# nauful/NLZM

Measured on AMD Instinct MI355X. Metric: compress MB/s, higher is better.
Workload: dtype u8; 1 GPU; enwik9 stand-in: 1000000000 B stream, -window:28; step = 41 launches of 8 chunks (40136704 B) of the stream; timed: bytes [200683520, 401367040) of 1000000000 (a prefix: the steps asked for end before the stream does); window_bits=28, batch_chunks=8, whole_stream=False

## Files before the change

### nlzm_amd/csrc/nlzm_core.h

```cpp
#pragma once

#include <stdint.h>

#ifndef NLZM_HD
#define NLZM_HD __host__ __device__ __forceinline__
#endif
#ifndef NLZM_HDN
#define NLZM_HDN __host__ __device__
#endif
#define NLZM_RARE(x) __builtin_expect(!!(x), 0)

namespace nlzm {

constexpr uint32_t kMatchMin = 2;
constexpr uint32_t kMatchMax = 264;
constexpr uint32_t kNice = 64;
constexpr uint32_t kParseMax = 4096;
constexpr uint32_t kNone = 0xFFFFFFFFu;

constexpr uint32_t kCtxCmd = 0;
constexpr uint32_t kCtxLitHi = 1;
constexpr uint32_t kCtxLitLo = 2;
constexpr uint32_t kCtxLenDirect = 18;
constexpr uint32_t kCtxLenExtHi = 19;
// ... 99 lines not shown
    uint32_t *cap_words; unsigned long long cap_cap, cap_lo, cap_hi; unsigned long long *cap_used;
    uint32_t workers;
    uint32_t batch_a0;
    uint32_t *bt_ready;
    uint32_t *bt_pairs;
    uint32_t bt_pstride;
    uint32_t *bt_ext;
    uint32_t *bt_ext_cur;
    uint32_t bt_ext_cap;
    uint32_t *bt_flag;
    const uint8_t *unc;
    const uint32_t *bin_off;
    const uint32_t *bin_pos;
    uint32_t nheads;
    uint32_t wthreads;
    const uint32_t *hot_of_bin;
    const uint32_t *hot_list;
    unsigned long long *hot_undo;
    uint32_t *bt_undo;
    uint32_t *abort_word;
    const uint32_t *progress;
    WorkerCounters *wcnt;
    uint32_t table_shape;
    uint32_t launch_par;
    uint32_t test_fail;
    void *hook_user;
};

NLZM_HD uint32_t match_min(uint32_t d)
{
// ... 131 lines not shown

struct BtView {
    const uint8_t *in;
    uint32_t *heads, *tree, *ready, *pairs;
    uint32_t batch_a0, bt_shift, wmask, tmask;
    uint32_t pstride = kBtMaxPairs;
    uint32_t *ext = nullptr, *ext_cur = nullptr;
    uint32_t ext_cap = 0;
    uint32_t *fail_word = nullptr;
};
NLZM_HD BtView bt_view(const Geom &g, const Globals &G)
{
    return BtView{ G.in, G.bt_heads, G.bt_tree, G.bt_ready, G.bt_pairs, G.batch_a0, g.bt_shift, g.wmask, g.bt_tmask,
                   G.bt_pstride, G.bt_ext, G.bt_ext_cur, G.bt_ext_cap, G.abort_word };
}
template <class IO>
NLZM_HD void ResultSink<IO>::operator()(uint32_t d, uint32_t l)
{
    if (!pairs || l <= best) return;
    best = l; best_d = d;
    const bool s0 = count == 0, s1 = count == 1, s2 = count == 2, s3 = count == 3;
    d0 = s0 ? d : d0; l0 = s0 ? l : l0; d1 = s1 ? d : d1; l1 = s1 ? l : l1;
    d2 = s2 ? d : d2; l2 = s2 ? l : l2; d3 = s3 ? d : d3; l3 = s3 ? l : l3;
    if (count >= 4) {
        uint32_t *q = bt_pair_ptr<IO>(pairs, view->pstride, view->ext, view->ext_cur, view->ext_cap, ext_idx, count);
        if (q) { IO::st_agent(q, d); IO::st_agent(q + 1, l); }
    }
    count++;
}

// ... 32 lines not shown
```

### nlzm_amd/csrc/nlzm_hip.cpp

```cpp
#include <hip/hip_runtime.h>
#include <dirent.h>
#include <unistd.h>

#include <stdarg.h>
#include <stdint.h>
#include <stdio.h>
#include <stdlib.h>
#include <string.h>

#include <array>
#include <mutex>
#include <thread>
#include <chrono>
#include <algorithm>
#include <vector>

#include "../../include/nlzm_hip.h"
#include "nlzm_core.h"
#include "nlzm_v2.h"

namespace nlzm {
void launch_rk_hash(const uint8_t *in, unsigned long long n, unsigned long long pos0, unsigned long long pos1,
                    uint32_t *out, hipStream_t st);
void launch_pipeline2(const Geom &g, const Globals &G, const v2::GlobalsV2 &V, uint32_t c0, uint32_t c1, uint32_t worker_blocks, hipStream_t st);
// ... 50 lines not shown
void blocks_close(DevState &D, bool drop_pool = false);
bool idle_block_pool_dropped();

inline uint32_t clampu(uint32_t v, uint32_t lo, uint32_t hi) { return v < lo ? lo : (v > hi ? hi : v); }

struct Pool {
    uint8_t *base = nullptr;
    size_t size = 0, used = 0;
    bool measuring = false;
};

struct Options {
    int64_t batch = 32;
    int64_t worker_blocks = 240;
    int64_t worker_threads = 128;
    int64_t hot_waves = 2;
    int64_t hot_min = 0;
    int64_t tbits_max = 34;
    int64_t block_threads = 320;
    int64_t block_hot_waves = 3;
    int64_t block_batch = 8;
    int64_t tbits_per = 4;
    int64_t keep_pool = 1;
    int64_t helper = 1;
    int64_t block_helper = 0;
    int64_t multi_same = 0;
    int64_t table_shape = 0;
    int64_t test_fail_launch = -1;
    int64_t test_fail_stream = 0;
    int64_t block_ext_blocks = -1;
    int64_t report = 0;
};

struct StreamConfig {
    bool in_set = false;
    uint32_t batch = 0;
    uint32_t worker_blocks = 0, worker_threads = 0;
    uint32_t nheads = 0;
    uint32_t hot_max = 0;
    uint32_t hot_min = 0;
    uint32_t t_bits = 0, m_bits = 0;
    uint32_t t_bitmap = 0;
    uint32_t pstride = kBtMaxPairs, ext_cap = 0;
    bool helper = false;
    uint32_t table_shape = 0;
    int64_t test_fail_launch = -1;
    unsigned long long rkhash_len = 0;
    unsigned long long syms_stride = 0, bits_stride = 0, frame_stride = 0;
};

struct LaunchSet {
    uint32_t *rkhash = nullptr, *bt_ready = nullptr, *bt_flag = nullptr, *abort_word = nullptr, *bin_off = nullptr, *bin_pos = nullptr,
// ... 225 lines not shown
    memset(&C.stats, 0, sizeof C.stats);
    memset(&C.tm, 0, sizeof C.tm);
    C.stats.in_bytes = n;
    StreamConfig &K = C.cfg;
    StreamBuffers &B = C.buf;
    K = StreamConfig{};
    K.in_set = C.pool != nullptr;
    K.batch = (uint32_t)(O.batch < 1 ? 1 : O.batch);
    if (g.nchunks && K.batch > g.nchunks) K.batch = g.nchunks;
    {
        const int64_t room = (int64_t)C.cu_count - (int64_t)pipeline2_role_blocks();
        if (room < 1) return set_err(NLZM_HIP_E_ARG, "device has %d CUs: the pipeline needs at least %u", C.cu_count, pipeline2_role_blocks() + 1);
        K.worker_blocks = (uint32_t)(O.worker_blocks > room ? room : (O.worker_blocks < 1 ? 1 : O.worker_blocks));
    }
    K.worker_threads = (uint32_t)O.worker_threads;
    {
        K.nheads = 1u << (32 - g.bt_shift);
        const unsigned long long lanes = (unsigned long long)K.worker_blocks * K.worker_threads;
        if (lanes < K.nheads) K.nheads = (uint32_t)lanes;
    }
    {
        int64_t hw = O.hot_waves;
        const int64_t spare = (512 - O.worker_threads) / 64;
        if (hw > spare) hw = spare;
        K.hot_max = hw > 0 ? (uint32_t)hw * K.worker_blocks : 0u;
    }
    K.hot_min = (uint32_t)O.hot_min; K.table_shape = (uint32_t)O.table_shape; K.test_fail_launch = O.test_fail_launch; K.helper = O.helper != 0;
    K.t_bits = prefilter_tbits(g, O.tbits_per, O.tbits_max);
    K.t_bitmap = prefilter_is_bitmap(g) ? 1u : 0u;
    K.pstride = K.in_set ? 32u : kBtMaxPairs;
// ... 115 lines not shown
    G.batch_a0 = (uint32_t)a0;
    {
        const unsigned long long lo = a0 > 1024 ? a0 - 1024 : 0;
        unsigned long long hi = a1 + g.feed + 256;
        if (hi + 255 > g.n) hi = g.n >= 255 ? g.n - 255 : 0;
        HIPCHK(hipEventRecord(ev[7], C.st));
        if (hi > lo && hi - lo > K.rkhash_len) return set_err(NLZM_HIP_E_ARG, "launch of %u chunks is larger than the stream was opened for", nb);
        G.rkhash = L.rkhash - lo;
        if (g.n >= 256 && hi > lo) launch_rk_hash(C.d_in, g.n, lo, hi, L.rkhash - lo, C.st);
    }
    HIPCHK(hipEventRecord(ev[5], C.st));
    {
        const unsigned long long cnt = a1 - a0;
        G.bt_ready = L.bt_ready; G.bt_pairs = B.bt_pairs; G.bt_flag = L.bt_flag; G.unc = L.unc;
        G.bt_pstride = K.pstride; G.bt_ext = B.bt_ext; G.bt_ext_cap = K.ext_cap; G.bt_ext_cur = &B.v2_hx->ext_cur;
        G.bin_off = L.bin_off; G.bin_pos = L.bin_pos; G.nheads = K.nheads; G.wthreads = K.worker_threads;
        G.abort_word = L.abort_word; G.wcnt = B.wcnt; G.bt_undo = B.bt_undo;
        HIPCHK(hipMemsetAsync(L.bt_ready, 0, cnt * 4 * kBtRec, C.st));
        HIPCHK(hipMemsetAsync(L.bt_flag, 0, cnt * 4, C.st));
        HIPCHK(hipMemsetAsync(L.abort_word, 0, 4, C.st));
        HIPCHK(hipMemsetAsync(L.bin_off, 0, (size_t)nb * (K.nheads + 1) * 4, C.st));
        launch_prefilter(C.d_in, g.n, (uint32_t)a0, (uint32_t)a1, g.wmask, K.t_bits, K.t_bitmap, K.m_bits, B.pf_T, B.pf_M, B.pf_h, B.pf_h2,
                         B.pf_c1, L.unc, C.st);
        launch_bin(C.d_in, g, c0, nb, K.nheads, L.bin_off, B.bin_cur, L.bin_pos, L.unc, (uint32_t)a0, C.st);
        if (K.hot_max) {
            const unsigned long long lpos = (unsigned long long)K.batch * g.chunk_size;
            const double by_pace = K.in_set ? (double)lpos / 480.0 : (C.last_launch_ms > 0 ? 24.0 * C.last_launch_ms : (double)lpos / 240.0);
            const uint32_t hot_min = K.hot_min > 0 ? K.hot_min : (uint32_t)(by_pace < 512 ? 512 : (by_pace > 1e9 ? 1e9 : by_pace));
            launch_hot_select(L.bin_off, nb, K.nheads, K.hot_max, hot_min, L.hot_of_bin, L.hot_list, B.wcnt, C.st);
            G.hot_of_bin = L.hot_of_bin; G.hot_list = L.hot_list; G.hot_undo = B.hot_undo;
        }
// ... 168 lines not shown
    fprintf(stderr, "finder: RK256 entries cut short by the uint16 length parameter that became the growing top entry: %llu; that ended exactly where another entry ends: %llu (%llu of them the nearer one)\n",
            P.prof[115], P.prof[116], P.prof[117]);
    fprintf(stderr, "finder: starts of nice regions whose segment the stage knew itself, ahead of the parser's word: %llu; that it had to wait for: %llu\n", P.prof[118], P.prof[119]);
    fprintf(stderr, "finder: worker results not there at the first look: %llu of positions whose call is the finder's decision (unc), %llu of others\n", P.prof[28], P.prof[29]);
    fprintf(stderr, "finder: blocks that had to wait for a worker result: %llu (%.0f cycles each); late results of hot bins' waves %llu, late results at lane 0 (the position the block before was cut at) %llu\n",
            P.prof[112], (double)P.prof[25] / (double)(P.prof[112] ? P.prof[112] : 1), P.prof[110], P.prof[111]);
    fprintf(stderr, "parser: waited for its record loader %llu times, the table stage %.0f positions ahead on average then\n", P.prof[26], (double)P.prof[27] / (double)(P.prof[26] ? P.prof[26] : 1));
    if (P.prof[96] || P.prof[100])
        fprintf(stderr, "helper parser: %llu jobs posted, %llu taken over (%llu nodes = %.1f %% of the positions), the parser stage waited %.0f cycles per position for it; "
                        "helper: %llu jobs seen, %llu done, %llu blocks (%.2f passes each), waited %.0f cycles per position for records\n",
                P.prof[96], P.prof[97], P.prof[98], 100.0 * P.prof[98] / n, P.prof[99] / n, P.prof[100], P.prof[101], P.prof[102],
                (double)P.prof[103] / (double)(P.prof[102] ? P.prof[102] : 1), P.prof[104] / n);
    if (P.prof[88]) fprintf(stderr, "finder sections (cycles/position, profile build): predict %.0f, own loads %.0f, HT rows %.0f, candidates + jobs %.0f, record + RK256 %.0f, "
                            "BT4 results (wait included) %.0f, verify %.0f, commit %.0f\n", P.prof[88] / n, P.prof[89] / n, P.prof[90] / n, P.prof[91] / n, P.prof[92] / n,
                            P.prof[93] / n, P.prof[94] / n, P.prof[95] / n);
    if (P.prof[44]) fprintf(stderr, "table stage sections (cycles/position summed over the waves, profile build): gather %.0f, scan %.0f, waiting for the carry %.0f, carry merge (the part in block order) %.0f, records %.0f\n",
                            P.prof[44] / n, P.prof[45] / n, P.prof[47] / n, P.prof[46] / n, P.prof[55] / n);
    if (P.prof[32]) {
        const double np = (double)(P.prof[13] ? P.prof[13] : 1);
        fprintf(stderr, "parser, cycles per pass (profile build): relax waves %.0f %.0f %.0f, probe wave %.0f (of it: sets that changed %.0f, mask fills %.0f), update %.0f, "
                        "barrier waits per wave %.0f %.0f %.0f %.0f; block end %.0f cycles/position\n",
                P.prof[32] / np, P.prof[33] / np, P.prof[34] / np, P.prof[35] / np, P.prof[43] / np, P.prof[41] / np, P.prof[40] / np,
                P.prof[36] / np, P.prof[37] / np, P.prof[38] / np, P.prof[39] / np, P.prof[42] / n);
        fprintf(stderr, "parser, cycles per pass by wave 0..7 (profile build): work");
        for (int w = 0; w < 8; w++) fprintf(stderr, " %.0f", P.prof[64 + w] / np);
        fprintf(stderr, " | barrier wait");
        for (int w = 0; w < 8; w++) fprintf(stderr, " %.0f", P.prof[72 + w] / np);
        fprintf(stderr, " | update");
        for (int w = 0; w < 8; w++) fprintf(stderr, " %.0f", P.prof[80 + w] / np);
        fprintf(stderr, "\n");
// ... 273 lines not shown

void nlzm_hip_block_placement(uint32_t nstreams, uint32_t blocks_per_stream, uint32_t workgroup, uint32_t *stream, uint32_t *local)
{
    uint32_t s = 0, l = 0;
    multi_block_of(nstreams * blocks_per_stream, blocks_per_stream, workgroup, s, l);
    if (stream) *stream = s;
    if (local) *local = l;
}

enum OptKind { kOptRange,
               kOptLanes,
               kOptFlag,
               kOptAny };
static const struct { const char *key; int64_t Options::*member; OptKind kind; int64_t lo, hi; } kOptions[] = {
    { "worker_blocks", &Options::worker_blocks, kOptRange, 1, 255 },
    { "hot_waves", &Options::hot_waves, kOptRange, 0, 6 },
    { "hot_min", &Options::hot_min, kOptRange, 0, 1 << 30 },
    { "worker_threads", &Options::worker_threads, kOptLanes, 64, 512 },
    { "block_worker_threads", &Options::block_threads, kOptLanes, 64, 512 },
    { "block_hot_waves", &Options::block_hot_waves, kOptRange, 0, 6 },
    { "prefilter_bits_per_position", &Options::tbits_per, kOptRange, 0, 8 },
    { "stage_report", &Options::report, kOptFlag, 0, 0 },
    { "parser_helper", &Options::helper, kOptFlag, 0, 0 },
    { "table_shape", &Options::table_shape, kOptRange, 0, 2 },
    { "multi_allow_same_device", &Options::multi_same, kOptFlag, 0, 0 },
    { "test_fail_launch", &Options::test_fail_launch, kOptAny, 0, 0 },
    { "test_fail_stream", &Options::test_fail_stream, kOptRange, 0, 63 },
    { "block_ext_blocks", &Options::block_ext_blocks, kOptAny, 0, 0 },
    { "block_parser_helper", &Options::block_helper, kOptFlag, 0, 0 },
    { "keep_block_pool", &Options::keep_pool, kOptFlag, 0, 0 },
// ... 779 lines not shown
```

### nlzm_amd/csrc/nlzm_kernels.hip

```cpp
#include <hip/hip_runtime.h>
#include <type_traits>
#include <cstddef>
#include <stdint.h>

#include "nlzm_core.h"
#include "nlzm_v2.h"

namespace nlzm {

#ifndef NLZM_LPW
#define NLZM_LPW 64
#endif
#ifndef NLZM_AHEAD
#define NLZM_AHEAD 3
#endif
constexpr uint32_t kAhead = NLZM_AHEAD;
constexpr uint32_t kEntryWords = 16;
union V2Lds {
    v2::FLds f; v2::TLds t; v2::PLds p;
    uint32_t wq[512 * kAhead * kEntryWords];
};
__shared__ V2Lds g_v2_lds;
}
namespace xw {
// ... 243 lines not shown
    }
    static __device__ __forceinline__ uint32_t ld_agent(const uint32_t *p)
    {
        return __hip_atomic_load(p, __ATOMIC_RELAXED, __HIP_MEMORY_SCOPE_AGENT);
    }
    static __device__ __forceinline__ uint32_t atomic_inc(uint32_t *p) { return __hip_atomic_fetch_add(p, 1u, __ATOMIC_RELAXED, __HIP_MEMORY_SCOPE_AGENT); }
    static __device__ __forceinline__ void drain() { asm volatile("s_waitcnt vmcnt(0)" ::: "memory"); }
    static __device__ __forceinline__ void st_quad(uint32_t *p, uint32_t a, uint32_t b, uint32_t c, uint32_t d)
    {
        typedef uint32_t u4 __attribute__((ext_vector_type(4)));
        const u4 v = { a, b, c, d };
        asm volatile("global_store_dwordx4 %0, %1, off sc1\n\ts_nop 1" :: "v"((__attribute__((address_space(1))) uint32_t *)p), "v"(v) : "memory");
    }
};

struct LaneSink {
    uint32_t *slot;
    uint32_t *pairs;
    uint32_t count = 0, best = 1, best_d = 0;
    uint32_t ext_idx = 0;
    __device__ __forceinline__ void put(const BtView &B, uint32_t d, uint32_t l)
    {
        best = l; best_d = d;
        if (count < 4) { slot[(2 * count) * 512] = d; slot[(2 * count + 1) * 512] = l; }
        else {
            uint32_t *q = bt_pair_ptr<LaneIO>(pairs, B.pstride, B.ext, B.ext_cur, B.ext_cap, ext_idx, count);
            if (q) { LaneIO::st_agent(q, d); LaneIO::st_agent(q + 1, l); }
        }
        count++;
    }
    __device__ __forceinline__ void publish(uint32_t *rec, uint32_t tests) const
    {
        if (count > 4) LaneIO::drain();
        const uint32_t d0 = count > 0 ? slot[0] : 0u, l0 = count > 0 ? slot[512] : 0u, d1 = count > 1 ? slot[2 * 512] : 0u, l1 = count > 1 ? slot[3 * 512] : 0u;
        const uint32_t d2 = count > 2 ? slot[4 * 512] : 0u, l2 = count > 2 ? slot[5 * 512] : 0u, d3 = count > 3 ? slot[6 * 512] : 0u, l3 = count > 3 ? slot[7 * 512] : 0u;
        LaneIO::st_quad(rec + 4, d0, l0, d1, kBtTag);
        LaneIO::st_quad(rec + 8, l1, d2, l2, kBtTag);
        LaneIO::st_quad(rec + 12, d3, l3, ext_idx, kBtTag);
        LaneIO::st_quad(rec, kBtReady | (tests << 9) | count, best_d, count ? best : 0u, 0u);
    }
};
constexpr uint32_t kUndoCap = 260;
__device__ __forceinline__ void bt_descent(const BtView &B, uint32_t a, uint32_t hidx, uint32_t max_len, bool keep, bool dry, uint32_t *undo,
                                           uint32_t &n_undo, LaneSink &sink, uint32_t &tests_out, uint32_t &cmp_out)
{
    const uint8_t *pa = B.in + a;
    uint32_t sp = B.heads[hidx];
    uint32_t nu = 0;
    if (keep) { *(unsigned long long *)undo = (0x80000000u | hidx) | ((unsigned long long)(dry ? a : sp) << 32); nu = 1; }
    if (!dry) B.heads[hidx] = a;
    uint32_t pend_l = (a & B.tmask) << 1, pend_r = pend_l + 1, len_l = 0, len_r = 0, tests = 0, cb = 0;
    uint32_t old_l = kNone, old_r = kNone;
    while (sp != kNone && a > sp && a - sp <= B.wmask && tests < 256) {
        tests++;
        const uint32_t pair = (sp & B.tmask) << 1;
        const uint8_t *ps = B.in + sp;
        const uint32_t init = umin(len_l, len_r);
        const unsigned long long pp = *(const unsigned long long *)(B.tree + pair);
        const unsigned long long x0 = load64u(ps + init), y0 = load64u(pa + init), d0 = x0 ^ y0;
        const unsigned long long x1 = load64u(ps + init + 8), y1 = load64u(pa + init + 8), d1 = x1 ^ y1;
        const uint32_t nb0 = d0 ? (uint32_t)__builtin_ctzll(d0) >> 3 : (d1 ? 8u + ((uint32_t)__builtin_ctzll(d1) >> 3) : 16u);
        uint32_t l = init + nb0;
        bool full = l >= max_len;
        const unsigned long long xs = nb0 < 8 ? x0 : x1, ys = nb0 < 8 ? y0 : y1;
        uint32_t sign = (uint32_t)(((xs >> (8 * (nb0 & 7u))) & 0xFF) < ((ys >> (8 * (nb0 & 7u))) & 0xFF));
        if (nb0 == 16 && !full) {
            for (;;) {
                const unsigned long long x = load64u(ps + l), y = load64u(pa + l), d = x ^ y;
                if (d) {
                    const uint32_t nb = (uint32_t)__builtin_ctzll(d) >> 3;
                    l += nb;
                    sign = (uint32_t)(((x >> (8 * nb)) & 0xFF) < ((y >> (8 * nb)) & 0xFF));
                    break;
                }
                l += 8;
                if (l >= max_len) break;
            }
            full = l >= max_len;
        }
        if (full) l = max_len;
        cb += (l - init) + (full ? 0u : 1u);
        const uint32_t pl = (uint32_t)pp, pr = (uint32_t)(pp >> 32), d = a - sp;
        if (l >= match_min(d) && l > sink.best) sink.put(B, d, l);
        if (full) {
            if (!dry) { B.tree[pend_l] = pl; B.tree[pend_r] = pr; }
            if (keep) {
                *(unsigned long long *)(undo + 2 * nu) = pend_l | ((unsigned long long)(dry ? pl : old_l) << 32);
                *(unsigned long long *)(undo + 2 * nu + 2) = pend_r | ((unsigned long long)(dry ? pr : old_r) << 32);
                nu += 2;
            }
            tests_out = tests; cmp_out = cb; n_undo = nu;
            return;
        }
        const bool right = sign != 0;
        const uint32_t slot = right ? pend_l : pend_r;
        if (!dry) B.tree[slot] = sp;
        if (keep) { *(unsigned long long *)(undo + 2 * nu) = slot | ((unsigned long long)(dry ? sp : (right ? old_l : old_r)) << 32); nu++; }
        pend_l = right ? pair + 1 : pend_l; pend_r = right ? pend_r : pair;
        old_l = right ? pr : old_l; old_r = right ? old_r : pl;
        len_r = right ? l : len_r; len_l = right ? len_l : l;
        sp = right ? pr : pl;
    }
    if (!dry) { B.tree[pend_r] = kNone; B.tree[pend_l] = kNone; }
    if (keep) {
        *(unsigned long long *)(undo + 2 * nu) = pend_r | ((unsigned long long)(dry ? kNone : old_r) << 32);
        *(unsigned long long *)(undo + 2 * nu + 2) = pend_l | ((unsigned long long)(dry ? kNone : old_l) << 32);
        nu += 2;
    }
    tests_out = tests; cmp_out = cb; n_undo = nu;
}

#ifndef NLZM_RISKY_AHEAD
#define NLZM_RISKY_AHEAD 0
#endif
constexpr uint32_t kPending = 0xFFFFFFFEu;
__device__ __forceinline__ uint32_t wave_max_u32(uint32_t v) { return (uint32_t)__builtin_amdgcn_readlane((int)xw::scan_max(v), 63); }
__device__ __forceinline__ void worker_role_hot(const Geom &g, const Globals &G, uint32_t c0, uint32_t c1, uint32_t bin, uint32_t hot_index)
{
    unsigned long long p0 = (unsigned long long)G.in, p1 = (unsigned long long)G.bt_heads, p2 = (unsigned long long)G.bt_tree,
                       p3 = (unsigned long long)G.bt_ready, p4 = (unsigned long long)G.bt_pairs, p5 = (unsigned long long)G.bt_flag,
                       p6 = (unsigned long long)G.hot_undo;
    uint32_t q0 = G.batch_a0, q2 = g.wmask, q3 = g.bt_tmask;
    asm volatile("" : "+s"(p0), "+s"(p1), "+s"(p2), "+s"(p3), "+s"(p4), "+s"(p5), "+s"(p6));
    asm volatile("" : "+s"(q0), "+s"(q2), "+s"(q3));
#define NLZM_AS_GLOBAL(T, x) ((T *)(__attribute__((address_space(1))) T *)(x))
// ... 355 lines not shown
    constexpr uint32_t kLpw = NLZM_LPW;
    const uint32_t lane_waves = (G.wthreads + kLpw - 1) / kLpw;
    if ((threadIdx.x >> 6) >= lane_waves) {
        if (!G.hot_list) return;
        const uint32_t k = ((threadIdx.x >> 6) - lane_waves) * wblocks + wblock;
        if (k >= G.hot_list[0]) return;
        worker_role_hot(g, G, c0, c1, G.hot_list[1 + k], k);
        return;
    }
    const uint32_t lane_in_block = (threadIdx.x >> 6) * kLpw + (threadIdx.x & 63u);
    const bool takes_bin = (threadIdx.x & 63u) < kLpw && lane_in_block < G.wthreads;
    const uint32_t gl = wblock * G.wthreads + (takes_bin ? lane_in_block : 0u);
    unsigned long long p0 = (unsigned long long)G.in, p1 = (unsigned long long)G.bt_heads, p2 = (unsigned long long)G.bt_tree,
                       p3 = (unsigned long long)G.bt_ready, p4 = (unsigned long long)G.bt_pairs;
    uint32_t q0 = G.batch_a0, q1 = g.bt_shift, q2 = g.wmask, q3 = g.bt_tmask;
    asm volatile("" : "+s"(p0), "+s"(p1), "+s"(p2), "+s"(p3), "+s"(p4));
    asm volatile("" : "+s"(q0), "+s"(q1), "+s"(q2), "+s"(q3));
#define NLZM_AS_GLOBAL(T, x) ((T *)(__attribute__((address_space(1))) T *)(x))
    BtView B{ NLZM_AS_GLOBAL(const uint8_t, p0), NLZM_AS_GLOBAL(uint32_t, p1), NLZM_AS_GLOBAL(uint32_t, p2), NLZM_AS_GLOBAL(uint32_t, p3),
              NLZM_AS_GLOBAL(uint32_t, p4), q0, q1, q2, q3 };
    B.pstride = G.bt_pstride; B.ext = G.bt_ext; B.ext_cur = G.bt_ext_cur; B.ext_cap = G.bt_ext_cap; B.fail_word = G.abort_word;
    uint32_t *const undo_base = NLZM_AS_GLOBAL(uint32_t, (unsigned long long)G.bt_undo) + (unsigned long long)gl * (kAhead * kUndoCap * 2);
#undef NLZM_AS_GLOBAL
    bool active = takes_bin && gl < G.nheads && !(G.hot_of_bin && G.hot_of_bin[gl < G.nheads ? gl : 0]);
    uint32_t c = c0;
    bool loaded = false;
    uint32_t i0 = 0, e0 = 0;
    uint32_t la_end = 0;
    unsigned long long n_calls = 0, n_tests = 0, n_cmp = 0, n_open = 0, n_wait = 0, n_cyc = 0, n_cyc_tests = 0, n_back = 0, n_redo = 0;
    uint32_t first = 0, nq = 0, head_a = 0;
    uint32_t *const my = (uint32_t *)&g_v2_lds + threadIdx.x;
    enum : uint32_t { kWa = 8, kWtests = 9, kWcmp = 10, kWcount = 11, kWbest = 12, kWbestd = 13, kWundo = 14, kWinfo = 15 };
    unsigned long long t_wait0 = 0;
    uint32_t idle = 0, prog_seen = 0;
    bool fail = false;

    while (__any(active)) {
        bool waiting = false;
        uint32_t job = 0, ja = 0, jh = 0, jlen = 0, jinfo = 0;
        if (active) {
            if (nq) {
                const uint32_t f = LaneIO::ld_agent(G.bt_flag + (head_a - G.batch_a0));
                const bool hdry = (my[(first * kEntryWords + kWinfo) * 512] >> 28) & 1u;
                if ((f == kFlagCall && !hdry) || (f == kFlagSkip && hdry)) {
                    for (uint32_t k = 0; k < kAhead; k++) {
                        uint32_t *e = my + (first * kEntryWords) * 512;
                        if (!((e[kWinfo * 512] >> 28) & 1u)) { n_calls++; n_tests += e[kWtests * 512]; n_cmp += e[kWcmp * 512]; }
                        first = first + 1 == kAhead ? 0u : first + 1; nq--;
                        if (!nq) break;
                        e = my + (first * kEntryWords) * 512;
                        const uint32_t ea = e[kWa * 512], einfo = e[kWinfo * 512];
                        if (!((einfo >> 28) & 1u)) {
                            LaneSink sk{ e, B.pairs + (unsigned long long)(ea - B.batch_a0) * (2 * B.pstride), e[kWcount * 512] & 0x1FFu, e[kWbest * 512], e[kWbestd * 512], e[kWcount * 512] >> 9 };
                            sk.publish(B.ready + (unsigned long long)(ea - B.batch_a0) * kBtRec, e[kWtests * 512]);
                        }
// ... 58 lines not shown
                }
            }
            if (!job && nq) {
                waiting = true;
                n_wait++;
                if ((++idle & 1023u) == 0) {
                    if (LaneIO::ld_agent(G.abort_word)) active = false;
                    const unsigned long long now = wall_clock64();
                    const uint32_t prog = G.progress ? LaneIO::ld_agent(G.progress) : 0u;
                    if (!t_wait0 || prog != prog_seen) { t_wait0 = now; prog_seen = prog; }
                    else if (now - t_wait0 > 3000000000ull) { fail = true; }
                }
            }
            if (fail) { LaneIO::st_agent(G.abort_word, 2u); active = false; job = 0; }
        }
        if (job) {
            const unsigned long long t0 = __builtin_readcyclecounter();
            const unsigned long long bi = ja - B.batch_a0;
            const uint32_t slot = first + nq >= kAhead ? first + nq - kAhead : first + nq;
            uint32_t *e = my + (slot * kEntryWords) * 512;
            LaneSink sink{ e, B.pairs + bi * (2 * B.pstride) };
            uint32_t tests = 0, cmpb = 0, nu = 0;
            const bool park = job == 2 && ((jinfo >> 28) & 1u);
            if (!park) bt_descent(B, ja, jh, jlen, job == 2, false, undo_base + slot * (kUndoCap * 2), nu, sink, tests, cmpb);
            if (job == 1) {
                sink.publish(B.ready + bi * kBtRec, tests);
                n_calls++; n_tests += tests; n_cmp += cmpb;
                n_cyc += __builtin_readcyclecounter() - t0; n_cyc_tests += tests;
            } else {
                if (!nq) { if (!park) sink.publish(B.ready + bi * kBtRec, tests); head_a = ja; t_wait0 = 0; idle = 0; }
                e[kWa * 512] = ja; e[kWtests * 512] = tests; e[kWcmp * 512] = cmpb; e[kWcount * 512] = sink.count | (sink.ext_idx << 9);
                e[kWbest * 512] = sink.best; e[kWbestd * 512] = sink.best_d; e[kWundo * 512] = nu; e[kWinfo * 512] = jinfo;
                nq++; if (!park) n_open++;
            }
        }
        if (!__any(active && !waiting)) __builtin_amdgcn_s_sleep(8);
    }
    if (nq) {
        atomicAdd(&G.wcnt->stuck_lanes, 1ull);
        atomicMax(&G.wcnt->stuck_pos_inv, (unsigned long long)(uint32_t)~head_a);
    }
    for (int m = 32; m >= 1; m >>= 1) {
        n_calls += __shfl_xor(n_calls, m, 64); n_tests += __shfl_xor(n_tests, m, 64); n_cmp += __shfl_xor(n_cmp, m, 64);
        n_open += __shfl_xor(n_open, m, 64); n_wait += __shfl_xor(n_wait, m, 64);
        n_cyc += __shfl_xor(n_cyc, m, 64); n_cyc_tests += __shfl_xor(n_cyc_tests, m, 64);
        n_back += __shfl_xor(n_back, m, 64); n_redo += __shfl_xor(n_redo, m, 64);
    }
    if ((threadIdx.x & 63) == 0) {
        atomicAdd(&G.wcnt->bt_calls, n_calls); atomicAdd(&G.wcnt->bt_tests, n_tests); atomicAdd(&G.wcnt->cmp_bytes, n_cmp);
// ... 243 lines not shown
```

### nlzm_amd/csrc/nlzm_v2.h

```cpp
#pragma once

#include "nlzm_core.h"
#include "xw.h"

namespace nlzm {
namespace v2 {

constexpr uint32_t kFtRing = 1u << 14;
constexpr uint32_t kFtStride = 16;
constexpr uint32_t kTpRing = 1u << 13;
constexpr uint32_t kMaxEdges = 32;
constexpr uint32_t kTpStride = 2 + 2 + 2 * kMaxEdges;
constexpr uint32_t kTpUniq = 2, kTpEdges = 4;
constexpr uint32_t kFrontMax = 264;
constexpr uint32_t kTfStride = 2 * kFrontMax;

constexpr uint32_t kFtBt = 8u, kFtTop = 16u;
struct Hx {
    alignas(128) uint32_t f_pos;
    alignas(128) uint32_t t_pos;
    alignas(128) uint32_t t_out;
    alignas(128) uint32_t p_pos;
    alignas(128) unsigned long long p_seg;
    alignas(128) uint32_t h_job;
// ... 122 lines not shown
    uint32_t reach_d = kNone;
    uint32_t s_active, s_d, s_end, s_seen;
    uint32_t rk_from, rk_to, rk_len, rk_end;
    uint32_t rk_cut = 0;
    uint32_t prev_nice, seg_s;
    uint32_t gap_last = 0;
    uint32_t n_seg_own = 0, n_seg_wait = 0;
    uint32_t t_pos_seen;
    uint32_t err;
    uint32_t dbg_a = 0;
    unsigned long long n_pos, n_nice, n_unc, n_ht, n_rkp, n_rki, n_cmp, n_blocks, n_cut0, n_cut1, n_cut2, n_cut3, n_cut4, n_cut5;
    unsigned long long n_cmp_lane = 0;
    unsigned long long t_wait, t_wait_bt = 0, t_total;
    uint32_t n_so_top = 0, n_so_tie = 0, n_so_won = 0;
    uint32_t n_late_unc = 0, n_late_other = 0, n_late_hot = 0, n_late_first = 0, n_late_blocks = 0;
    unsigned long long t_f[8] = {};
#ifdef NLZM_PROFILE
    XW_FN unsigned long long ptick() const { return xw::tick(); }
#else
    XW_FN unsigned long long ptick() const { return 0; }
#endif

    XW_FN void fail(uint32_t code, uint32_t pos, uint32_t site = 0, uint32_t x0 = 0, uint32_t x1 = 0)
    {
        err = code;
        if (xw::lane() == 0) raise(V.hx, code, kStFinder, site, pos, x0, x1);
    }

    uint32_t pend_fpos = 0;
    uint32_t pf_a0 = kNone, pf_rkh = 0;
// ... 299 lines not shown
        uint32_t bt_n = 0;
        flush_fpos();
        const uint32_t ec0 = ec, ec_d0 = ec_d, od0 = od;
        uint32_t pm = 0, before = 0, js = 64, jo = 64, cut_nice = 64, m = 0;
        bool nice_real = false, so_top = false, so_tie = false, so_win = false;
        unsigned long long stm = 0, om = 0;
        {
            const unsigned long long tw = xw::tick();
            const unsigned long long t0 = xw::clock100();
            uint32_t spins = 0;
            const bool waits = xw::any(bt_wait);
            bool have = !bt_wait;
            uint32_t r_d = 0, r_l = 0;
            bool told = false;
            uint32_t f_seen = 65;
            for (;;) {
                {
                    const unsigned long long ask = xw::ballot(!have);
                    if (ask && i == (uint32_t)__builtin_ctzll(ask)) xw::need_bt(G.hook_user, a);
                }
                if (!have) {
                    const xw::u32x4 q0 = xw::ld_agent128(G.bt_ready + bi * kBtRec);
                    if (q0.x & kBtReady) { have = true; bt_n = q0.x & 0x1FFu; r_d = q0.y; r_l = q0.z; }
                }
                const unsigned long long missing = xw::ballot(!have);
                if (waits && spins == 0) {
                    n_late_unc += (uint32_t)__builtin_popcountll(missing & xw::ballot(unc));
                    n_late_other += (uint32_t)__builtin_popcountll(missing & ~xw::ballot(unc));
                    if (missing) {
                        const bool hot = G.hot_of_bin && !have && G.hot_of_bin[(hash4(v4) >> g.bt_shift) % G.nheads] != 0;
                        n_late_hot += (uint32_t)__builtin_popcountll(xw::ballot(hot));
                        n_late_first += (uint32_t)(missing & 1ull);
                        n_late_blocks++;
                    }
                }
                const uint32_t F = missing ? (uint32_t)__builtin_ctzll(missing) : 64u;
                if (F != f_seen) {
                    f_seen = F;
                    xw::after_poll();
                    ec = ec0; ec_d = ec_d0; od = od0;
                    if (bt_wait && have && bt_n) { if (r_l >= cap) od = umin(od, r_d); else closed_end(a + r_l, r_d); }
                    pm = xw::scan_max(in_blk ? umax(ec, so_end) : 0u);
                    before = umax(xw::lane_below(pm, 0u), reach);
                    if (i >= jc && s_active) before = umax(before, s_end);
                    nice_real = in_blk && umax(before, s_sliding ? s_e : 0u) >= a + kNice;
                    const bool so_free = in_blk && so_end != 0 && od == kNone && !s_sliding;
                    so_tie = so_free && so_end == umax(before, ec);
                    so_win = false;
                    if (xw::any(so_tie)) {
                        uint32_t d2 = kNone;
                        if (ec == so_end) d2 = ec_d;
// ... 23 lines not shown
                    if (xw::readfirst(xw::ld_agent(&V.hx->err))) { err = kErrInternal + 100; return 1; }
#ifndef NLZM_SIM
                    if (xw::clock100() - t0 > 3000000000ull) {
                        const uint32_t fl = (uint32_t)__builtin_ctzll(missing | (1ull << 63));
                        fail(kErrTimeout, a0 + fl, 6, (uint32_t)__builtin_popcountll(missing) | (xw::readlane(unc ? 1u : 0u, fl) << 8) | (n << 16),
                             xw::readlane((hash4(v4) >> g.bt_shift) % G.nheads, fl));
                        return 1;
                    }
#else
                    (void)t0;
#endif
                }
                xw::pause();
            }
            if (waits) { t_wait += xw::tick() - tw; t_wait_bt += xw::tick() - tw; }
        }

        const unsigned long long f6 = ptick();
        if (m == 0) { fail(kErrInternal, a0, 7); return 1; }
        n_blocks++;
        if (m < n) {
            const uint32_t w = m == cut_nice ? 0u : (m == jo + 1 ? 1u : (m == cut_ev ? 2u : (m == cut_rk ? 3u : (m == cut_bin ? 5u : 4u))));
            n_cut0 += w == 0; n_cut1 += w == 1; n_cut2 += w == 2; n_cut3 += w == 3; n_cut4 += w == 4; n_cut5 += w == 5;
        }
        const bool fin = i < m;
        {
            const unsigned long long gapm = xw::ballot(fin && umax(before, s_sliding ? s_e : 0u) <= a);
            if (gapm) gap_last = a0 + (63u - (uint32_t)__builtin_clzll(gapm));
        }
        if (stm || xw::any(so_tie)) {
// ... 140 lines not shown
            xw::atomic_add64_agent(&c.positions, n_pos); xw::atomic_add64_agent(&c.nice_positions, n_nice);
            xw::atomic_add64_agent(&c.uncertain_positions, n_unc); xw::atomic_add64_agent(&c.ht_rows, 3 * n_ht);
            xw::atomic_add64_agent(&c.rk_probes, n_rkp); xw::atomic_add64_agent(&c.rk_inserts, n_rki);
            xw::atomic_add64_agent(&c.cmp_bytes, n_cmp); xw::atomic_add64_agent(&c.shifts, shifts);
            unsigned long long *pr = P->prof;
            xw::atomic_add64_agent(&pr[0], n_blocks); xw::atomic_add64_agent(&pr[1], n_cut0); xw::atomic_add64_agent(&pr[2], n_cut1);
            xw::atomic_add64_agent(&pr[3], n_cut2); xw::atomic_add64_agent(&pr[4], n_cut3); xw::atomic_add64_agent(&pr[5], n_cut4);
            xw::atomic_add64_agent(&pr[12], n_cut5);
            xw::atomic_add64_agent(&pr[16], t_wait); xw::atomic_add64_agent(&pr[17], xw::tick() - t_start); xw::atomic_add64_agent(&pr[25], t_wait_bt);
            xw::atomic_add64_agent(&pr[28], n_late_unc); xw::atomic_add64_agent(&pr[29], n_late_other);
            xw::atomic_add64_agent(&pr[115], n_so_top); xw::atomic_add64_agent(&pr[116], n_so_tie); xw::atomic_add64_agent(&pr[117], n_so_won);
            xw::atomic_add64_agent(&pr[118], n_seg_own); xw::atomic_add64_agent(&pr[119], n_seg_wait);
            xw::atomic_add64_agent(&pr[110], n_late_hot); xw::atomic_add64_agent(&pr[111], n_late_first); xw::atomic_add64_agent(&pr[112], n_late_blocks);
#ifdef NLZM_PROFILE
            for (int z = 0; z < 8; z++) xw::atomic_add64_agent(&pr[88 + z], t_f[z]);
#endif
            if (err || xw::ld_agent(&V.hx->err)) {
                uint32_t *d = V.hx->dbg[0];
                xw::st_agent(d + 0, dbg_a); xw::st_agent(d + 1, reach); xw::st_agent(d + 2, s_active); xw::st_agent(d + 3, s_d);
                xw::st_agent(d + 4, s_end); xw::st_agent(d + 5, prev_nice); xw::st_agent(d + 6, seg_s); xw::st_agent(d + 7, rk_len);
                xw::st_agent(d + 8, t_pos_seen); xw::st_agent(d + 9, err); xw::st_agent(d + 10, base);
            }
        }
    }
};


#ifndef NLZM_FRCAP
#define NLZM_FRCAP 16
#endif
// ... 1574 lines not shown
```

Before: 6.633 MB/s.

## Make worker binary-tree descent resumable in bounded slices between job polls

Splits the per-lane binary-tree descent into start, a bounded run of tests, and an end step, keeping descent state across loop iterations so a lane can pause mid-descent. A new worker_slice option caps tests per iteration, intended to reduce wave divergence where one long descent stalls the other lanes. With the default of 0 the slice is unlimited, so the loop behaves like the old single-shot descent but carries extra state and branching. The change also adds profile-build counters that split finder wait time by lane versus hot-bin owner.

```diff
diff --git a/nlzm_amd/csrc/nlzm_core.h b/nlzm_amd/csrc/nlzm_core.h
--- a/nlzm_amd/csrc/nlzm_core.h
+++ b/nlzm_amd/csrc/nlzm_core.h
@@ -137,6 +137,7 @@
     const uint32_t *bin_pos;
     uint32_t nheads;
     uint32_t wthreads;
+    uint32_t worker_slice;
     const uint32_t *hot_of_bin;
     const uint32_t *hot_list;
     unsigned long long *hot_undo;
@@ -298,6 +299,135 @@
     return BtView{ G.in, G.bt_heads, G.bt_tree, G.bt_ready, G.bt_pairs, G.batch_a0, g.bt_shift, g.wmask, g.bt_tmask,
                    G.bt_pstride, G.bt_ext, G.bt_ext_cur, G.bt_ext_cap, G.abort_word };
 }
+template <class IO, uint32_t kStride>
+struct SlotSink {
+    uint32_t *slot;
+    uint32_t *pairs;
+    uint32_t count = 0, best = 1, best_d = 0;
+    uint32_t ext_idx = 0;
+    NLZM_HD void put(const BtView &B, uint32_t d, uint32_t l)
+    {
+        best = l; best_d = d;
+        if (count < 4) { slot[(2 * count) * kStride] = d; slot[(2 * count + 1) * kStride] = l; }
+        else {
+            uint32_t *q = bt_pair_ptr<IO>(pairs, B.pstride, B.ext, B.ext_cur, B.ext_cap, ext_idx, count);
+            if (q) { IO::st_agent(q, d); IO::st_agent(q + 1, l); }
+        }
+        count++;
+    }
+    NLZM_HD void publish(uint32_t *rec, uint32_t tests) const
+    {
+        if (count > 4) IO::drain();
+        const uint32_t d0 = count > 0 ? slot[0] : 0u, l0 = count > 0 ? slot[kStride] : 0u, d1 = count > 1 ? slot[2 * kStride] : 0u, l1 = count > 1 ? slot[3 * kStride] : 0u;
+        const uint32_t d2 = count > 2 ? slot[4 * kStride] : 0u, l2 = count > 2 ? slot[5 * kStride] : 0u, d3 = count > 3 ? slot[6 * kStride] : 0u, l3 = count > 3 ? slot[7 * kStride] : 0u;
+        IO::st_quad(rec + 4, d0, l0, d1, kBtTag);
+        IO::st_quad(rec + 8, l1, d2, l2, kBtTag);
+        IO::st_quad(rec + 12, d3, l3, ext_idx, kBtTag);
+        IO::st_quad(rec, kBtReady | (tests << 9) | count, best_d, count ? best : 0u, 0u);
+    }
+};
+constexpr uint32_t kUndoCap = 260;
+struct BtCall {
+    uint32_t sp;
+    uint32_t pend_l, pend_r;
+    uint32_t len_l, len_r;
+    uint32_t old_l, old_r;
+    uint32_t tests, cb, nu;
+};
+enum : uint32_t { kBtMore = 0,
+                  kBtEndLeaf = 1,
+                  kBtEndFull = 2 };
+NLZM_HD void bt_call_start(const BtView &B, BtCall &s, uint32_t a, uint32_t hidx, bool keep, bool dry, uint32_t *undo)
+{
+    s.sp = B.heads[hidx];
+    s.nu = 0;
+    if (keep) { *(unsigned long long *)undo = (0x80000000u | hidx) | ((unsigned long long)(dry ? a : s.sp) << 32); s.nu = 1; }
+    if (!dry) B.heads[hidx] = a;
+    s.pend_l = (a & B.tmask) << 1; s.pend_r = s.pend_l + 1; s.len_l = 0; s.len_r = 0; s.tests = 0; s.cb = 0;
+    s.old_l = kNone; s.old_r = kNone;
+}
+template <class Sink>
+NLZM_HD uint32_t bt_call_tests(const BtView &B, BtCall &s, uint32_t a, uint32_t max_len, bool keep, bool dry, uint32_t *undo, Sink &sink,
+                               uint32_t budget, uint32_t &pl_out, uint32_t &pr_out)
+{
+    const uint8_t *pa = B.in + a;
+    uint32_t sp = s.sp, pend_l = s.pend_l, pend_r = s.pend_r, len_l = s.len_l, len_r = s.len_r, old_l = s.old_l, old_r = s.old_r;
+    uint32_t tests = s.tests, cb = s.cb, nu = s.nu, how = kBtEndLeaf;
+    while (sp != kNone && a > sp && a - sp <= B.wmask && tests < 256) {
+        if (!budget) { how = kBtMore; break; }
+        budget--;
+        tests++;
+        const uint32_t pair = (sp & B.tmask) << 1;
+        const uint8_t *ps = B.in + sp;
+        const uint32_t init = umin(len_l, len_r);
+        const unsigned long long pp = *(const unsigned long long *)(B.tree + pair);
+        const unsigned long long x0 = load64u(ps + init), y0 = load64u(pa + init), d0 = x0 ^ y0;
+        const unsigned long long x1 = load64u(ps + init + 8), y1 = load64u(pa + init + 8), d1 = x1 ^ y1;
+        const uint32_t nb0 = d0 ? (uint32_t)__builtin_ctzll(d0) >> 3 : (d1 ? 8u + ((uint32_t)__builtin_ctzll(d1) >> 3) : 16u);
+        uint32_t l = init + nb0;
+        bool full = l >= max_len;
+        const unsigned long long xs = nb0 < 8 ? x0 : x1, ys = nb0 < 8 ? y0 : y1;
+        uint32_t sign = (uint32_t)(((xs >> (8 * (nb0 & 7u))) & 0xFF) < ((ys >> (8 * (nb0 & 7u))) & 0xFF));
+        if (nb0 == 16 && !full) {
+            for (;;) {
+                const unsigned long long x = load64u(ps + l), y = load64u(pa + l), d = x ^ y;
+                if (d) {
+                    const uint32_t nb = (uint32_t)__builtin_ctzll(d) >> 3;
+                    l += nb;
+                    sign = (uint32_t)(((x >> (8 * nb)) & 0xFF) < ((y >> (8 * nb)) & 0xFF));
+                    break;
+                }
+                l += 8;
+                if (l >= max_len) break;
+            }
+            full = l >= max_len;
+        }
+        if (full) l = max_len;
+        cb += (l - init) + (full ? 0u : 1u);
+        const uint32_t pl = (uint32_t)pp, pr = (uint32_t)(pp >> 32), d = a - sp;
+        if (l >= match_min(d) && l > sink.best) sink.put(B, d, l);
+        if (full) { pl_out = pl; pr_out = pr; how = kBtEndFull; break; }
+        const bool right = sign != 0;
+        const uint32_t slot = right ? pend_l : pend_r;
+        if (!dry) B.tree[slot] = sp;
+        if (keep) { *(unsigned long long *)(undo + 2 * nu) = slot | ((unsigned long long)(dry ? sp : (right ? old_l : old_r)) << 32); nu++; }
+        pend_l = right ? pair + 1 : pend_l; pend_r = right ? pend_r : pair;
+        old_l = right ? pr : old_l; old_r = right ? old_r : pl;
+        len_r = right ? l : len_r; len_l = right ? len_l : l;
+        sp = right ? pr : pl;
+    }
+    s.sp = sp; s.pend_l = pend_l; s.pend_r = pend_r; s.len_l = len_l; s.len_r = len_r; s.old_l = old_l; s.old_r = old_r;
+    s.tests = tests; s.cb = cb; s.nu = nu;
+    return how;
+}
+NLZM_HD void bt_call_end(const BtView &B, BtCall &s, uint32_t how, uint32_t pl, uint32_t pr, bool keep, bool dry, uint32_t *undo)
+{
+    if (how == kBtEndFull) {
+        if (!dry) { B.tree[s.pend_l] = pl; B.tree[s.pend_r] = pr; }
+        if (keep) {
+            *(unsigned long long *)(undo + 2 * s.nu) = s.pend_l | ((unsigned long long)(dry ? pl : s.old_l) << 32);
+            *(unsigned long long *)(undo + 2 * s.nu + 2) = s.pend_r | ((unsigned long long)(dry ? pr : s.old_r) << 32);
+            s.nu += 2;
+        }
+        return;
+    }
+    if (!dry) { B.tree[s.pend_r] = kNone; B.tree[s.pend_l] = kNone; }
+    if (keep) {
+        *(unsigned long long *)(undo + 2 * s.nu) = s.pend_r | ((unsigned long long)(dry ? kNone : s.old_r) << 32);
+        *(unsigned long long *)(undo + 2 * s.nu + 2) = s.pend_l | ((unsigned long long)(dry ? kNone : s.old_l) << 32);
+        s.nu += 2;
+    }
+}
+template <class Sink>
+NLZM_HD bool bt_call_slice(const BtView &B, BtCall &s, uint32_t a, uint32_t max_len, bool keep, bool dry, uint32_t *undo, Sink &sink, uint32_t budget)
+{
+    uint32_t pl = 0, pr = 0;
+    const uint32_t how = bt_call_tests(B, s, a, max_len, keep, dry, undo, sink, budget, pl, pr);
+    if (how == kBtMore) return false;
+    bt_call_end(B, s, how, pl, pr, keep, dry, undo);
+    return true;
+}
+
 template <class IO>
 NLZM_HD void ResultSink<IO>::operator()(uint32_t d, uint32_t l)
 {
diff --git a/nlzm_amd/csrc/nlzm_hip.cpp b/nlzm_amd/csrc/nlzm_hip.cpp
--- a/nlzm_amd/csrc/nlzm_hip.cpp
+++ b/nlzm_amd/csrc/nlzm_hip.cpp
@@ -88,6 +88,7 @@
     int64_t batch = 32;
     int64_t worker_blocks = 240;
     int64_t worker_threads = 128;
+    int64_t worker_slice = 0;
     int64_t hot_waves = 2;
     int64_t hot_min = 0;
     int64_t tbits_max = 34;
@@ -110,6 +111,7 @@
     bool in_set = false;
     uint32_t batch = 0;
     uint32_t worker_blocks = 0, worker_threads = 0;
+    uint32_t worker_slice = 0;
     uint32_t nheads = 0;
     uint32_t hot_max = 0;
     uint32_t hot_min = 0;
@@ -365,6 +367,7 @@
         K.worker_blocks = (uint32_t)(O.worker_blocks > room ? room : (O.worker_blocks < 1 ? 1 : O.worker_blocks));
     }
     K.worker_threads = (uint32_t)O.worker_threads;
+    K.worker_slice = (uint32_t)O.worker_slice;
     {
         K.nheads = 1u << (32 - g.bt_shift);
         const unsigned long long lanes = (unsigned long long)K.worker_blocks * K.worker_threads;
@@ -510,7 +513,7 @@
         const unsigned long long cnt = a1 - a0;
         G.bt_ready = L.bt_ready; G.bt_pairs = B.bt_pairs; G.bt_flag = L.bt_flag; G.unc = L.unc;
         G.bt_pstride = K.pstride; G.bt_ext = B.bt_ext; G.bt_ext_cap = K.ext_cap; G.bt_ext_cur = &B.v2_hx->ext_cur;
-        G.bin_off = L.bin_off; G.bin_pos = L.bin_pos; G.nheads = K.nheads; G.wthreads = K.worker_threads;
+        G.bin_off = L.bin_off; G.bin_pos = L.bin_pos; G.nheads = K.nheads; G.wthreads = K.worker_threads; G.worker_slice = K.worker_slice;
         G.abort_word = L.abort_word; G.wcnt = B.wcnt; G.bt_undo = B.bt_undo;
         HIPCHK(hipMemsetAsync(L.bt_ready, 0, cnt * 4 * kBtRec, C.st));
         HIPCHK(hipMemsetAsync(L.bt_flag, 0, cnt * 4, C.st));
@@ -709,6 +712,9 @@
     if (P.prof[88]) fprintf(stderr, "finder sections (cycles/position, profile build): predict %.0f, own loads %.0f, HT rows %.0f, candidates + jobs %.0f, record + RK256 %.0f, "
                             "BT4 results (wait included) %.0f, verify %.0f, commit %.0f\n", P.prof[88] / n, P.prof[89] / n, P.prof[90] / n, P.prof[91] / n, P.prof[92] / n,
                             P.prof[93] / n, P.prof[94] / n, P.prof[95] / n);
+    if (P.prof[88]) fprintf(stderr, "finder: the wait for worker results by whose result the first missing lane of the block was waiting for (cycles/position, profile build): "
+                            "a lane's %.1f, a hot bin's wave's %.1f, neither (the last look, the verification) %.1f\n", P.prof[120] / n, P.prof[121] / n,
+                            ((double)P.prof[25] - (double)P.prof[120] - (double)P.prof[121]) / n);
     if (P.prof[44]) fprintf(stderr, "table stage sections (cycles/position summed over the waves, profile build): gather %.0f, scan %.0f, waiting for the carry %.0f, carry merge (the part in block order) %.0f, records %.0f\n",
                             P.prof[44] / n, P.prof[45] / n, P.prof[47] / n, P.prof[46] / n, P.prof[55] / n);
     if (P.prof[32]) {
@@ -1012,6 +1018,7 @@
                kOptAny };
 static const struct { const char *key; int64_t Options::*member; OptKind kind; int64_t lo, hi; } kOptions[] = {
     { "worker_blocks", &Options::worker_blocks, kOptRange, 1, 255 },
+    { "worker_slice", &Options::worker_slice, kOptRange, 0, 256 },
     { "hot_waves", &Options::hot_waves, kOptRange, 0, 6 },
     { "hot_min", &Options::hot_min, kOptRange, 0, 1 << 30 },
     { "worker_threads", &Options::worker_threads, kOptLanes, 64, 512 },
diff --git a/nlzm_amd/csrc/nlzm_kernels.hip b/nlzm_amd/csrc/nlzm_kernels.hip
--- a/nlzm_amd/csrc/nlzm_kernels.hip
+++ b/nlzm_amd/csrc/nlzm_kernels.hip
@@ -281,101 +281,7 @@
     }
 };
 
-struct LaneSink {
-    uint32_t *slot;
-    uint32_t *pairs;
-    uint32_t count = 0, best = 1, best_d = 0;
-    uint32_t ext_idx = 0;
-    __device__ __forceinline__ void put(const BtView &B, uint32_t d, uint32_t l)
-    {
-        best = l; best_d = d;
-        if (count < 4) { slot[(2 * count) * 512] = d; slot[(2 * count + 1) * 512] = l; }
-        else {
-            uint32_t *q = bt_pair_ptr<LaneIO>(pairs, B.pstride, B.ext, B.ext_cur, B.ext_cap, ext_idx, count);
-            if (q) { LaneIO::st_agent(q, d); LaneIO::st_agent(q + 1, l); }
-        }
-        count++;
-    }
-    __device__ __forceinline__ void publish(uint32_t *rec, uint32_t tests) const
-    {
-        if (count > 4) LaneIO::drain();
-        const uint32_t d0 = count > 0 ? slot[0] : 0u, l0 = count > 0 ? slot[512] : 0u, d1 = count > 1 ? slot[2 * 512] : 0u, l1 = count > 1 ? slot[3 * 512] : 0u;
-        const uint32_t d2 = count > 2 ? slot[4 * 512] : 0u, l2 = count > 2 ? slot[5 * 512] : 0u, d3 = count > 3 ? slot[6 * 512] : 0u, l3 = count > 3 ? slot[7 * 512] : 0u;
-        LaneIO::st_quad(rec + 4, d0, l0, d1, kBtTag);
-        LaneIO::st_quad(rec + 8, l1, d2, l2, kBtTag);
-        LaneIO::st_quad(rec + 12, d3, l3, ext_idx, kBtTag);
-        LaneIO::st_quad(rec, kBtReady | (tests << 9) | count, best_d, count ? best : 0u, 0u);
-    }
-};
-constexpr uint32_t kUndoCap = 260;
-__device__ __forceinline__ void bt_descent(const BtView &B, uint32_t a, uint32_t hidx, uint32_t max_len, bool keep, bool dry, uint32_t *undo,
-                                           uint32_t &n_undo, LaneSink &sink, uint32_t &tests_out, uint32_t &cmp_out)
-{
-    const uint8_t *pa = B.in + a;
-    uint32_t sp = B.heads[hidx];
-    uint32_t nu = 0;
-    if (keep) { *(unsigned long long *)undo = (0x80000000u | hidx) | ((unsigned long long)(dry ? a : sp) << 32); nu = 1; }
-    if (!dry) B.heads[hidx] = a;
-    uint32_t pend_l = (a & B.tmask) << 1, pend_r = pend_l + 1, len_l = 0, len_r = 0, tests = 0, cb = 0;
-    uint32_t old_l = kNone, old_r = kNone;
-    while (sp != kNone && a > sp && a - sp <= B.wmask && tests < 256) {
-        tests++;
-        const uint32_t pair = (sp & B.tmask) << 1;
-        const uint8_t *ps = B.in + sp;
-        const uint32_t init = umin(len_l, len_r);
-        const unsigned long long pp = *(const unsigned long long *)(B.tree + pair);
-        const unsigned long long x0 = load64u(ps + init), y0 = load64u(pa + init), d0 = x0 ^ y0;
-        const unsigned long long x1 = load64u(ps + init + 8), y1 = load64u(pa + init + 8), d1 = x1 ^ y1;
-        const uint32_t nb0 = d0 ? (uint32_t)__builtin_ctzll(d0) >> 3 : (d1 ? 8u + ((uint32_t)__builtin_ctzll(d1) >> 3) : 16u);
-        uint32_t l = init + nb0;
-        bool full = l >= max_len;
-        const unsigned long long xs = nb0 < 8 ? x0 : x1, ys = nb0 < 8 ? y0 : y1;
-        uint32_t sign = (uint32_t)(((xs >> (8 * (nb0 & 7u))) & 0xFF) < ((ys >> (8 * (nb0 & 7u))) & 0xFF));
-        if (nb0 == 16 && !full) {
-            for (;;) {
-                const unsigned long long x = load64u(ps + l), y = load64u(pa + l), d = x ^ y;
-                if (d) {
-                    const uint32_t nb = (uint32_t)__builtin_ctzll(d) >> 3;
-                    l += nb;
-                    sign = (uint32_t)(((x >> (8 * nb)) & 0xFF) < ((y >> (8 * nb)) & 0xFF));
-                    break;
-                }
-                l += 8;
-                if (l >= max_len) break;
-            }
-            full = l >= max_len;
-        }
-        if (full) l = max_len;
-        cb += (l - init) + (full ? 0u : 1u);
-        const uint32_t pl = (uint32_t)pp, pr = (uint32_t)(pp >> 32), d = a - sp;
-        if (l >= match_min(d) && l > sink.best) sink.put(B, d, l);
-        if (full) {
-            if (!dry) { B.tree[pend_l] = pl; B.tree[pend_r] = pr; }
-            if (keep) {
-                *(unsigned long long *)(undo + 2 * nu) = pend_l | ((unsigned long long)(dry ? pl : old_l) << 32);
-                *(unsigned long long *)(undo + 2 * nu + 2) = pend_r | ((unsigned long long)(dry ? pr : old_r) << 32);
-                nu += 2;
-            }
-            tests_out = tests; cmp_out = cb; n_undo = nu;
-            return;
-        }
-        const bool right = sign != 0;
-        const uint32_t slot = right ? pend_l : pend_r;
-        if (!dry) B.tree[slot] = sp;
-        if (keep) { *(unsigned long long *)(undo + 2 * nu) = slot | ((unsigned long long)(dry ? sp : (right ? old_l : old_r)) << 32); nu++; }
-        pend_l = right ? pair + 1 : pend_l; pend_r = right ? pend_r : pair;
-        old_l = right ? pr : old_l; old_r = right ? old_r : pl;
-        len_r = right ? l : len_r; len_l = right ? len_l : l;
-        sp = right ? pr : pl;
-    }
-    if (!dry) { B.tree[pend_r] = kNone; B.tree[pend_l] = kNone; }
-    if (keep) {
-        *(unsigned long long *)(undo + 2 * nu) = pend_r | ((unsigned long long)(dry ? kNone : old_r) << 32);
-        *(unsigned long long *)(undo + 2 * nu + 2) = pend_l | ((unsigned long long)(dry ? kNone : old_l) << 32);
-        nu += 2;
-    }
-    tests_out = tests; cmp_out = cb; n_undo = nu;
-}
+using LaneSink = SlotSink<LaneIO, 512>;
 
 #ifndef NLZM_RISKY_AHEAD
 #define NLZM_RISKY_AHEAD 0
@@ -761,8 +667,9 @@
     unsigned long long p0 = (unsigned long long)G.in, p1 = (unsigned long long)G.bt_heads, p2 = (unsigned long long)G.bt_tree,
                        p3 = (unsigned long long)G.bt_ready, p4 = (unsigned long long)G.bt_pairs;
     uint32_t q0 = G.batch_a0, q1 = g.bt_shift, q2 = g.wmask, q3 = g.bt_tmask;
+    uint32_t slice = G.worker_slice ? G.worker_slice : 0xFFFFFFFFu;
     asm volatile("" : "+s"(p0), "+s"(p1), "+s"(p2), "+s"(p3), "+s"(p4));
-    asm volatile("" : "+s"(q0), "+s"(q1), "+s"(q2), "+s"(q3));
+    asm volatile("" : "+s"(q0), "+s"(q1), "+s"(q2), "+s"(q3), "+s"(slice));
 #define NLZM_AS_GLOBAL(T, x) ((T *)(__attribute__((address_space(1))) T *)(x))
     BtView B{ NLZM_AS_GLOBAL(const uint8_t, p0), NLZM_AS_GLOBAL(uint32_t, p1), NLZM_AS_GLOBAL(uint32_t, p2), NLZM_AS_GLOBAL(uint32_t, p3),
               NLZM_AS_GLOBAL(uint32_t, p4), q0, q1, q2, q3 };
@@ -781,11 +688,15 @@
     unsigned long long t_wait0 = 0;
     uint32_t idle = 0, prog_seen = 0;
     bool fail = false;
+    uint32_t busy = 0, ca = 0, clen = 0, cinfo = 0;
+    uint32_t s_count = 0, s_best = 1, s_best_d = 0, s_ext = 0;
+    BtCall cs{};
+    unsigned long long c_cyc = 0;
 
     while (__any(active)) {
         bool waiting = false;
         uint32_t job = 0, ja = 0, jh = 0, jlen = 0, jinfo = 0;
-        if (active) {
+        if (active && !busy) {
             if (nq) {
                 const uint32_t f = LaneIO::ld_agent(G.bt_flag + (head_a - G.batch_a0));
                 const bool hdry = (my[(first * kEntryWords + kWinfo) * 512] >> 28) & 1u;
@@ -874,25 +785,44 @@
             }
             if (fail) { LaneIO::st_agent(G.abort_word, 2u); active = false; job = 0; }
         }
+        const uint32_t slot = first + nq >= kAhead ? first + nq - kAhead : first + nq;
+        uint32_t *const e = my + (slot * kEntryWords) * 512;
+        uint32_t *const undo = undo_base + slot * (kUndoCap * 2);
+        bool ended = false;
         if (job) {
+            const bool park = job == 2 && ((jinfo >> 28) & 1u);
+            ca = ja; clen = jlen; cinfo = jinfo;
+            s_count = 0; s_best = 1; s_best_d = 0; s_ext = 0;
+            cs.tests = 0; cs.cb = 0; cs.nu = 0;
+            if (park) { busy = job; ended = true; c_cyc = 0; }
+            else {
+                const unsigned long long t0 = __builtin_readcyclecounter();
+                bt_call_start(B, cs, ja, jh, job == 2, false, undo);
+                busy = job;
+                c_cyc = __builtin_readcyclecounter() - t0;
+            }
+        }
+        if (busy) {
             const unsigned long long t0 = __builtin_readcyclecounter();
-            const unsigned long long bi = ja - B.batch_a0;
-            const uint32_t slot = first + nq >= kAhead ? first + nq - kAhead : first + nq;
-            uint32_t *e = my + (slot * kEntryWords) * 512;
-            LaneSink sink{ e, B.pairs + bi * (2 * B.pstride) };
-            uint32_t tests = 0, cmpb = 0, nu = 0;
-            const bool park = job == 2 && ((jinfo >> 28) & 1u);
-            if (!park) bt_descent(B, ja, jh, jlen, job == 2, false, undo_base + slot * (kUndoCap * 2), nu, sink, tests, cmpb);
-            if (job == 1) {
-                sink.publish(B.ready + bi * kBtRec, tests);
-                n_calls++; n_tests += tests; n_cmp += cmpb;
-                n_cyc += __builtin_readcyclecounter() - t0; n_cyc_tests += tests;
-            } else {
-                if (!nq) { if (!park) sink.publish(B.ready + bi * kBtRec, tests); head_a = ja; t_wait0 = 0; idle = 0; }
-                e[kWa * 512] = ja; e[kWtests * 512] = tests; e[kWcmp * 512] = cmpb; e[kWcount * 512] = sink.count | (sink.ext_idx << 9);
-                e[kWbest * 512] = sink.best; e[kWbestd * 512] = sink.best_d; e[kWundo * 512] = nu; e[kWinfo * 512] = jinfo;
-                nq++; if (!park) n_open++;
-            }
+            const unsigned long long bi = ca - B.batch_a0;
+            LaneSink sink{ e, B.pairs + bi * (2 * B.pstride), s_count, s_best, s_best_d, s_ext };
+            const bool park = ended;
+            if (!park) ended = bt_call_slice(B, cs, ca, clen, busy == 2, false, undo, sink, slice);
+            s_count = sink.count; s_best = sink.best; s_best_d = sink.best_d; s_ext = sink.ext_idx;
+            if (ended) {
+                const uint32_t tests = cs.tests, cmpb = cs.cb, nu = cs.nu;
+                if (busy == 1) {
+                    sink.publish(B.ready + bi * kBtRec, tests);
+                    n_calls++; n_tests += tests; n_cmp += cmpb;
+                    n_cyc += c_cyc + (__builtin_readcyclecounter() - t0); n_cyc_tests += tests;
+                } else {
+                    if (!nq) { if (!park) sink.publish(B.ready + bi * kBtRec, tests); head_a = ca; t_wait0 = 0; idle = 0; }
+                    e[kWa * 512] = ca; e[kWtests * 512] = tests; e[kWcmp * 512] = cmpb; e[kWcount * 512] = sink.count | (sink.ext_idx << 9);
+                    e[kWbest * 512] = sink.best; e[kWbestd * 512] = sink.best_d; e[kWundo * 512] = nu; e[kWinfo * 512] = cinfo;
+                    nq++; if (!park) n_open++;
+                }
+                busy = 0;
+            } else c_cyc += __builtin_readcyclecounter() - t0;
         }
         if (!__any(active && !waiting)) __builtin_amdgcn_s_sleep(8);
     }
diff --git a/nlzm_amd/csrc/nlzm_v2.h b/nlzm_amd/csrc/nlzm_v2.h
--- a/nlzm_amd/csrc/nlzm_v2.h
+++ b/nlzm_amd/csrc/nlzm_v2.h
@@ -160,6 +160,7 @@
     unsigned long long t_wait, t_wait_bt = 0, t_total;
     uint32_t n_so_top = 0, n_so_tie = 0, n_so_won = 0;
     uint32_t n_late_unc = 0, n_late_other = 0, n_late_hot = 0, n_late_first = 0, n_late_blocks = 0;
+    unsigned long long t_wait_lane = 0, t_wait_hot = 0;
     unsigned long long t_f[8] = {};
 #ifdef NLZM_PROFILE
     XW_FN unsigned long long ptick() const { return xw::tick(); }
@@ -489,6 +490,11 @@
             uint32_t r_d = 0, r_l = 0;
             bool told = false;
             uint32_t f_seen = 65;
+#ifdef NLZM_PROFILE
+            const bool hot_me = bt_wait && G.hot_of_bin && G.hot_of_bin[(hash4(v4) >> g.bt_shift) % G.nheads] != 0;
+            unsigned long long tp = tw;
+            uint32_t owner = 0;
+#endif
             for (;;) {
                 {
                     const unsigned long long ask = xw::ballot(!have);
@@ -510,6 +516,14 @@
                     }
                 }
                 const uint32_t F = missing ? (uint32_t)__builtin_ctzll(missing) : 64u;
+#ifdef NLZM_PROFILE
+                if (waits) {
+                    const unsigned long long now = xw::tick();
+                    if (owner == 1) t_wait_lane += now - tp; else if (owner == 2) t_wait_hot += now - tp;
+                    tp = now;
+                    owner = F < 64 ? (xw::readlane(hot_me ? 1u : 0u, F) ? 2u : 1u) : 0u;
+                }
+#endif
                 if (F != f_seen) {
                     f_seen = F;
                     xw::after_poll();
@@ -563,6 +577,9 @@
                 xw::pause();
             }
             if (waits) { t_wait += xw::tick() - tw; t_wait_bt += xw::tick() - tw; }
+#ifdef NLZM_PROFILE
+            if (waits) { const unsigned long long now = xw::tick(); if (owner == 1) t_wait_lane += now - tp; else if (owner == 2) t_wait_hot += now - tp; }
+#endif
         }
 
         const unsigned long long f6 = ptick();
@@ -733,6 +750,7 @@
             xw::atomic_add64_agent(&pr[110], n_late_hot); xw::atomic_add64_agent(&pr[111], n_late_first); xw::atomic_add64_agent(&pr[112], n_late_blocks);
 #ifdef NLZM_PROFILE
             for (int z = 0; z < 8; z++) xw::atomic_add64_agent(&pr[88 + z], t_f[z]);
+            xw::atomic_add64_agent(&pr[120], t_wait_lane); xw::atomic_add64_agent(&pr[121], t_wait_hot);
 #endif
             if (err || xw::ld_agent(&V.hx->err)) {
                 uint32_t *d = V.hx->dbg[0];
```

Result: no change. 6.647 MB/s, median of 6 (+0.2%).
